# wondmgezahu/RAMP

Measured on AMD Instinct MI355X. Metric: sampled trajectories/sec (H=48, T=25), higher is better.
Workload: dtype f32-emulated (2 x fp16 planes per operand, fp32 accumulate)

## Files before the change

### ramp_amd/csrc/tkc.hip

```cpp
#include "args_conv.h"
#include "tokmma.h"

#include <algorithm>

namespace ramp {

namespace {

constexpr int tc_xrows(int NG) { return NG == 4 ? 64 + 2 + 2 : 48 + 2 * 6 + 2; }
constexpr int tc_scr(int NG) { return NG == 4 ? 2304 : 2048; }

__device__ __forceinline__ float tc_mish(float x) {
  const float e = __builtin_amdgcn_exp2f(fminf(x, 20.f) * 1.44269504088896340736f);
  const float n = e * (e + 2.f);
  return x * (n * __builtin_amdgcn_rcpf(n + 2.f));
}
__device__ __forceinline__ float tc_mish_grad(float x) {
  const float e = __builtin_amdgcn_exp2f(fminf(x, 20.f) * 1.44269504088896340736f);
  const float n = e * (e + 2.f);
  const float w = __builtin_amdgcn_rcpf(n + 2.f);
  return n * w + x * (4.f * e * (e + 1.f) * w * w);
}

__device__ __forceinline__ f32x4 tc_mm32(const u32x4 a, const u32x4 b, const f32x4 c) {
  return __builtin_amdgcn_mfma_f32_16x16x32_f16(__builtin_bit_cast(half8, a), __builtin_bit_cast(half8, b), c, 0, 0, 0);
}
__device__ __forceinline__ void tc_wave_sync() {
  __builtin_amdgcn_fence(__ATOMIC_ACQ_REL, "wavefront");
  __builtin_amdgcn_wave_barrier();
}

}

__global__ void tkc_pack_kernel(const float* __restrict__ W, unsigned short* __restrict__ out, int N, int K, float scale) {
  const int total = 5 * (N / 16) * (K / 32) * 64;
  const int idx = blockIdx.x * 256 + threadIdx.x;
  if (idx >= total) return;
  const int lane = idx & 63, f = idx >> 6;
  const int j = f % (K / 32), nb = (f / (K / 32)) % (N / 16), tap = f / ((K / 32) * (N / 16));
  const float* src = W + ((long)tap * N + 16 * nb + (lane & 15)) * K + 32 * j + 8 * (lane >> 4);
  unsigned short* o = out + (long)f * 1024 + lane * 8;
#pragma unroll
  for (int e = 0; e < 8; ++e) {
    const float x = src[e] * scale;
    const _Float16 hi = (_Float16)x, lo = (_Float16)(x - (float)hi);
    o[e] = __builtin_bit_cast(unsigned short, hi); o[512 + e] = __builtin_bit_cast(unsigned short, lo);
  }
}
int tkc_pack(const float* W, int N, int K, float scale, unsigned short* out, hipStream_t s) {
  RAMP_REQUIRE(W && out && N % 16 == 0 && K % 32 == 0 && N >= 16 && N <= 64 && K >= 32 && K <= 64, "tkc_pack: bad shape");
  const int total = 5 * (N / 16) * (K / 32) * 64;
  hipLaunchKernelGGL(tkc_pack_kernel, dim3((total + 255) / 256), dim3(256), 0, s, W, out, N, K, scale);
  RAMP_HIP_CHECK(hipGetLastError());
  return 0;
}
size_t tkc_packed_halves(int N, int K) { return (size_t)5 * (N / 16) * (K / 32) * 1024; }

template <int NG, int NB, int KS, int PRO, int EPI>
__global__ __launch_bounds__(256) __attribute__((amdgpu_waves_per_eu(1, 2)))
void tkc_kernel(TkcArgs a, int n_tiles) {
  constexpr int T = 16 * NG, K = 32 * KS, N = 16 * NB;
  constexpr int XROW = 4 * K + 16;
  constexpr int WBYTES = 5 * NB * KS * 2048;
  constexpr int TC_XROWS = tc_xrows(NG), TC_SCR = tc_scr(NG);
  static_assert(8 * T * 4 + 8 * (NG == 4 ? 1 : 6) * 4 <= TC_SCR, "GroupNorm scratch");
  extern __shared__ __attribute__((aligned(16))) char smem[];
  const int tid = threadIdx.x, lane = tid & 63;
  const int wave = __builtin_amdgcn_readfirstlane(tid >> 6);
  const int c = lane & 15, g = lane >> 4;
  const int n_my = (n_tiles - (int)blockIdx.x + (int)gridDim.x - 1) / (int)gridDim.x;

  const bool exact = a.amax_in == nullptr;
  float s_in = scale_of(a.amax_in);
  float os = a.wsi / s_in;
  float amax = 0.f;

  for (int i = tid; i < WBYTES / 16; i += 256) reinterpret_cast<u32x4*>(smem)[i] = reinterpret_cast<const u32x4*>(a.W)[i];
  char* xt = smem + WBYTES + wave * (TC_XROWS * XROW);
  for (int i = lane; i < TC_XROWS * XROW / 16; i += 64) reinterpret_cast<u32x4*>(xt)[i] = u32x4{0u, 0u, 0u, 0u};
  float* const wscr = reinterpret_cast<float*>(smem + WBYTES + 4 * (TC_XROWS * XROW) + wave * TC_SCR);
  __syncthreads();

  int xrow[NG], smp[NG];
#pragma unroll
  for (int t = 0; t < NG; ++t) { smp[t] = (16 * t + c) / a.L; xrow[t] = (16 * t + c) + 2 * smp[t] + 2; }
  const int n_smp = T / a.L;
  auto tok_sums = [&](float (&v)[4][NG], int nblk, int C) __attribute__((always_inline)) {
    const int gsz = C >> 3;
#pragma unroll
    for (int b = 0; b < 4; ++b) {
      if (b < nblk) {
#pragma unroll
        for (int t = 0; t < NG; ++t) {
          float q = v[b][t];
          if (gsz == 8) q += __shfl_xor(q, 16);
          const int grp = gsz == 4 ? 4 * b + g : 2 * b + (g >> 1);
          if (gsz == 4 || !(g & 1)) wscr[grp * T + 16 * t + c] = q;
        }
      }
    }
    tc_wave_sync();
    if (lane < 8 * n_smp) {
      const int grp = lane / n_smp, sm = lane - grp * n_smp;
      double q = 0.0;
      for (int u = 0; u < a.L; ++u) q += (double)wscr[grp * T + sm * a.L + u];
      wscr[8 * T + lane] = (float)(q / (double)(a.L * gsz));
    }
    tc_wave_sync();
#pragma unroll
    for (int b = 0; b < 4; ++b) {
      if (b < nblk) {
#pragma unroll
        for (int t = 0; t < NG; ++t) {
          const int grp = gsz == 4 ? 4 * b + g : 2 * b + (g >> 1);
          v[b][t] = wscr[8 * T + grp * n_smp + smp[t]];
        }
      }
    }
    tc_wave_sync();
  };
  const int m_last = a.M - 1;
  const char* xbase = reinterpret_cast<const char*>(a.X);

  f32x4 xr[K / 16][NG];
  f32x4 cr[PRO ? K / 16 : 1][PRO ? NG : 1];
  float gmu[PRO ? K / 16 : 1][PRO ? NG : 1], grs[PRO ? K / 16 : 1][PRO ? NG : 1];
  auto load_x = [&](int tile) __attribute__((always_inline)) {
    int tk0 = tile * (4 * T) + wave * T + c;
    asm volatile("" : "+v"(tk0));
#pragma unroll
    for (int t = 0; t < NG; ++t) {
      const unsigned tk = (unsigned)min(tk0 + 16 * t, m_last);
      const char* row = xbase + ((size_t)tk * (unsigned)(4 * a.ldx) + 16u * (unsigned)g);
#pragma unroll
      for (int fb = 0; fb < K / 16; ++fb) xr[fb][t] = *reinterpret_cast<const f32x4*>(row + 64 * fb);
      if constexpr (PRO) {
        const char* crow = reinterpret_cast<const char*>(a.gn_c) + ((size_t)tk * (unsigned)(4 * K) + 16u * (unsigned)g);
        const unsigned srow = tk / (unsigned)a.L;
// ... 13 lines not shown
      pgam[fb] = *reinterpret_cast<const f32x4*>(a.gn_gamma + 16 * fb + 4 * g); pbet[fb] = *reinterpret_cast<const f32x4*>(a.gn_beta + 16 * fb + 4 * g);
    }
  }
  load_x((int)blockIdx.x);

#pragma unroll 1
  for (int ti = 0; ti < n_my; ++ti) {
    const int tile = (int)blockIdx.x + ti * (int)gridDim.x;
    const int tile_n = ti + 1 < n_my ? tile + (int)gridDim.x : tile;
    const int tok0 = tile * (4 * T) + wave * T;
    const bool full = tok0 + T <= a.M;

    if constexpr (PRO) {
      float v1[4][NG], v2[4][NG];
#pragma unroll
      for (int fb = 0; fb < K / 16; ++fb)
#pragma unroll
        for (int t = 0; t < NG; ++t) {
          float s1 = 0.f, s2 = 0.f;
#pragma unroll
          for (int j = 0; j < 4; ++j) {
            const float h = (cr[fb][t][j] - gmu[fb][t]) * grs[fb][t];
            const float d = xr[fb][t][j] * tc_mish_grad(h * pgam[fb][j] + pbet[fb][j]) * pgam[fb][j];
            cr[fb][t][j] = h; xr[fb][t][j] = d;
            s1 += d; s2 += d * h;
          }
          v1[fb][t] = s1; v2[fb][t] = s2;
        }
      tok_sums(v1, K / 16, K);
      tok_sums(v2, K / 16, K);
#pragma unroll
      for (int fb = 0; fb < K / 16; ++fb)
#pragma unroll
        for (int t = 0; t < NG; ++t)
#pragma unroll
          for (int j = 0; j < 4; ++j) xr[fb][t][j] = (xr[fb][t][j] - v1[fb][t] - cr[fb][t][j] * v2[fb][t]) * grs[fb][t];
    }
    if (exact) {
      float tm = 0.f;
#pragma unroll
      for (int t = 0; t < NG; ++t) {
        const float lm = (full || tok0 + 16 * t + c < a.M) ? 1.f : 0.f;
#pragma unroll
        for (int fb = 0; fb < K / 16; ++fb) tm = amax4(xr[fb][t] * lm, tm);
      }
      tm = fmaxf(tm, __shfl_xor(tm, 32)); tm = fmaxf(tm, __shfl_xor(tm, 16)); tm = fmaxf(tm, __shfl_xor(tm, 8));
      tm = fmaxf(tm, __shfl_xor(tm, 4)); tm = fmaxf(tm, __shfl_xor(tm, 2)); tm = fmaxf(tm, __shfl_xor(tm, 1));
      s_in = scale_from(tm);
      os = a.wsi / s_in;
    }
#pragma unroll
    for (int t = 0; t < NG; ++t) {
      const float lm = (full || tok0 + 16 * t + c < a.M) ? 1.f : 0.f;
      char* dst = xt + xrow[t] * XROW + 8 * g;
#pragma unroll
      for (int fb = 0; fb < K / 16; ++fb) {
        const f32x4 v = xr[fb][t] * lm;
        amax = amax4(v, amax);
        unsigned h0, h1, l0, l1;
        split4(v * s_in, h0, h1, l0, l1);
        *reinterpret_cast<u32x2*>(dst + 32 * fb) = u32x2{h0, h1};
        *reinterpret_cast<u32x2*>(dst + 2 * K + 32 * fb) = u32x2{l0, l1};
      }
    }
    tc_wave_sync();
    load_x(tile_n);

    f32x4 acc[NB][NG];
#pragma unroll
    for (int nb = 0; nb < NB; ++nb)
#pragma unroll
      for (int t = 0; t < NG; ++t) acc[nb][t] = f32x4{0.f, 0.f, 0.f, 0.f};
#pragma unroll
    for (int tap = 0; tap < 5; ++tap) {
      const int sh = a.dir * (tap - 2);
#pragma unroll
      for (int j = 0; j < KS; ++j) {
        u32x4 bh[NG], bl[NG];
#pragma unroll
        for (int t = 0; t < NG; ++t) {
          const char* p = xt + (xrow[t] + sh) * XROW + 64 * j + 16 * g;
          bh[t] = *reinterpret_cast<const u32x4*>(p);
          bl[t] = *reinterpret_cast<const u32x4*>(p + 2 * K);
        }
#pragma unroll
        for (int nb = 0; nb < NB; ++nb) {
          const char* wp = smem + ((tap * NB + nb) * KS + j) * 2048 + lane * 16;
          const u32x4 wh = *reinterpret_cast<const u32x4*>(wp), wl = *reinterpret_cast<const u32x4*>(wp + 1024);
#pragma unroll
          for (int t = 0; t < NG; ++t) {
            f32x4 v = acc[nb][t];
            v = tc_mm32(wh, bl[t], v);
            v = tc_mm32(wl, bh[t], v);
            v = tc_mm32(wh, bh[t], v);
            acc[nb][t] = v;
          }
        }
      }
    }
    tc_wave_sync();

    if constexpr (EPI) {
      unsigned trow[NG];
#pragma unroll
      for (int t = 0; t < NG; ++t) trow[t] = (unsigned)min(tok0 + 16 * t + c, m_last);
      const float* tline[EPI == 2 ? NG : 1];
      if constexpr (EPI == 2) {
        const int s0 = tok0 / a.L, s_last = a.M / a.L - 1;
#pragma unroll
        for (int t = 0; t < NG; ++t) tline[t] = a.tbias + (size_t)a.t_rows[min(s0 + smp[t], s_last)] * (size_t)a.tt_stride + 4 * g;
      }
      float mean[4][NG], var[4][NG];
#pragma unroll
      for (int nb = 0; nb < NB; ++nb) {
        const f32x4 bq = *reinterpret_cast<const f32x4*>(a.bias + 16 * nb + 4 * g);
#pragma unroll
        for (int t = 0; t < NG; ++t) {
          acc[nb][t] = acc[nb][t] * os + bq;
          if (full || tok0 + 16 * t + c < a.M) *reinterpret_cast<f32x4*>(a.Cst + (size_t)trow[t] * N + 16 * nb + 4 * g) = acc[nb][t];
          mean[nb][t] = (acc[nb][t][0] + acc[nb][t][1]) + (acc[nb][t][2] + acc[nb][t][3]);
        }
      }
      tok_sums(mean, NB, N);
#pragma unroll
      for (int nb = 0; nb < NB; ++nb)
#pragma unroll
        for (int t = 0; t < NG; ++t) {
          float q = 0.f;
#pragma unroll
          for (int j = 0; j < 4; ++j) { const float d = acc[nb][t][j] - mean[nb][t]; q += d * d; }
          var[nb][t] = q;
        }
      tok_sums(var, NB, N);
#pragma unroll
// ... 26 lines not shown
#pragma unroll
      for (int nb = 0; nb < NB; ++nb) bq[nb] = a.bias ? *reinterpret_cast<const f32x4*>(a.bias + 16 * nb + 4 * g) : f32x4{0.f, 0.f, 0.f, 0.f};
      if (full) {
        f32x4 rz[NB][NG];
#pragma unroll
        for (int nb = 0; nb < NB; ++nb)
#pragma unroll
          for (int t = 0; t < NG; ++t) rz[nb][t] = f32x4{0.f, 0.f, 0.f, 0.f};
        if (a.resid) {
#pragma unroll
          for (int nb = 0; nb < NB; ++nb)
#pragma unroll
            for (int t = 0; t < NG; ++t) rz[nb][t] = *reinterpret_cast<const f32x4*>(a.resid + (size_t)trow[t] * a.ldr + 16 * nb + 4 * g);
        }
        if (a.resid2) {
#pragma unroll
          for (int nb = 0; nb < NB; ++nb)
#pragma unroll
            for (int t = 0; t < NG; ++t) rz[nb][t] += *reinterpret_cast<const f32x4*>(a.resid2 + (size_t)trow[t] * a.ldr2 + 16 * nb + 4 * g);
        }
#pragma unroll
        for (int nb = 0; nb < NB; ++nb)
#pragma unroll
          for (int t = 0; t < NG; ++t) *reinterpret_cast<f32x4*>(a.Y + (size_t)trow[t] * a.ldy + 16 * nb + 4 * g) = acc[nb][t] * os + bq[nb] + rz[nb][t];
      } else {
#pragma unroll
        for (int nb = 0; nb < NB; ++nb)
#pragma unroll
          for (int t = 0; t < NG; ++t) {
            f32x4 v = acc[nb][t] * os + bq[nb];
            if (a.resid) v += *reinterpret_cast<const f32x4*>(a.resid + (size_t)trow[t] * a.ldr + 16 * nb + 4 * g);
            if (a.resid2) v += *reinterpret_cast<const f32x4*>(a.resid2 + (size_t)trow[t] * a.ldr2 + 16 * nb + 4 * g);
            if (tok0 + 16 * t + c < a.M) *reinterpret_cast<f32x4*>(a.Y + (size_t)trow[t] * a.ldy + 16 * nb + 4 * g) = v;
          }
      }
    }
  }

    }
  amax = fmaxf(amax, __shfl_xor(amax, 32)); amax = fmaxf(amax, __shfl_xor(amax, 16)); amax = fmaxf(amax, __shfl_xor(amax, 8));
  amax = fmaxf(amax, __shfl_xor(amax, 4)); amax = fmaxf(amax, __shfl_xor(amax, 2)); amax = fmaxf(amax, __shfl_xor(amax, 1));
  __syncthreads();
  record_amax_block_guarded<true>(a.amax_out, amax, reinterpret_cast<float*>(smem + WBYTES), exact ? nullptr : a.range_flag, s_in, a.site);
}

bool tkc_applicable(int M, int L, int N, int K, int* ng) {
  int n = 0;
  if (L >= 8 && 48 % L == 0) n = 3; else if (L >= 8 && 32 % L == 0) n = 2; else if (L == 64 && !(N == 64 && K == 64)) n = 4;
  if (ng) *ng = n;
  return n != 0 && M > 0 && M % L == 0 && (N == 32 || N == 64) && (K == 32 || K == 64);
}

namespace {
template <int NG, int NB, int KS> size_t tkc_lds() { return (size_t)5 * NB * KS * 2048 + 4 * (size_t)tc_xrows(NG) * (4 * 32 * KS + 16) + 4 * tc_scr(NG); }
template <int NG, int NB, int KS, int PRO, int EPI> int tkc_go(const TkcArgs& a, int n_tiles, hipStream_t s) {
  const size_t lds = tkc_lds<NG, NB, KS>();
  const int per_cu = lds * 2 <= 160 * 1024 ? 2 : 1;
  const int nb = std::min(n_tiles, per_cu * device_cu_count());
  hipLaunchKernelGGL((tkc_kernel<NG, NB, KS, PRO, EPI>), dim3(nb), dim3(256), lds, s, a, n_tiles);
  RAMP_HIP_CHECK(hipGetLastError());
  return 0;
}
}

int launch_tkc(const TkcArgs& a, hipStream_t s) {
  auto al16 = [](const void* p) { return (reinterpret_cast<uintptr_t>(p) & 15) == 0; };
  int ng = 0;
  RAMP_REQUIRE(tkc_applicable(a.M, a.L, a.N, a.K, &ng), "tkc: C_in, C_out in {32, 64}, tokens per sample >= 8 dividing 48 or 32 (or 64, not 64 x 64 channels), whole samples");
  RAMP_REQUIRE(a.X && a.W && a.Y && (a.dir == 1 || a.dir == -1), "tkc: bad operand");
  RAMP_REQUIRE(al16(a.X) && al16(a.W) && al16(a.Y) && al16(a.bias) && al16(a.resid) && al16(a.resid2) && a.ldx % 4 == 0 && a.ldy % 4 == 0 &&
               a.ldr % 4 == 0 && a.ldr2 % 4 == 0 && a.ldx >= a.K && a.ldy >= a.N, "tkc: operands must be 16-byte aligned");
  RAMP_REQUIRE((long)a.M * a.ldx * 4 < (1l << 32), "tkc: 32-bit row offsets");
  RAMP_REQUIRE(!ranges_overlap(a.Y, ((size_t)(a.M - 1) * a.ldy + a.N) * 4, a.X, ((size_t)(a.M - 1) * a.ldx + a.K) * 4), "tkc: the output must not overlap the operand");
  const int T = 16 * ng, n_tiles = (a.M + 4 * T - 1) / (4 * T);
  const int pro = a.gn_c ? 1 : 0, epi = a.Cst ? (a.t_rows ? 2 : 1) : 0;
  RAMP_REQUIRE(!a.t_rows || (a.Cst && a.tbias && a.tt_stride > 0 && a.tt_stride % 4 == 0), "tkc: a row -> timestep table needs the GroupNorm epilogue, the time table and its stride (a multiple of 4 floats)");
  RAMP_REQUIRE(!(pro && epi), "tkc: the GroupNorm backward operand and the GroupNorm epilogue do not occur together");
  if (pro) RAMP_REQUIRE(a.gn_stats && a.gn_gamma && a.gn_beta && al16(a.gn_c) && al16(a.gn_gamma) && al16(a.gn_beta) && a.ldx >= a.K, "tkc: GroupNorm-backward operand incomplete");
  if (epi) RAMP_REQUIRE(a.stats && a.gamma && a.beta && a.bias && !a.resid2 && al16(a.Cst) && al16(a.gamma) && al16(a.beta) && al16(a.tbias), "tkc: GroupNorm epilogue incomplete");
#define TC_SHAPE(NGV, PROV, EPIV) \
    if (a.N == 64 && a.K == 64) return tkc_go<NGV, 4, 2, PROV, EPIV>(a, n_tiles, s); \
    if (a.N == 64 && a.K == 32) return tkc_go<NGV, 4, 1, PROV, EPIV>(a, n_tiles, s); \
    if (a.N == 32 && a.K == 64) return tkc_go<NGV, 2, 2, PROV, EPIV>(a, n_tiles, s); \
    return tkc_go<NGV, 2, 1, PROV, EPIV>(a, n_tiles, s);
#define TC_CASE(NGV) \
  if (ng == NGV) { \
    if (pro) { TC_SHAPE(NGV, 1, 0) } \
    if (epi == 2) { TC_SHAPE(NGV, 0, 2) } \
    if (epi) { TC_SHAPE(NGV, 0, 1) } \
    TC_SHAPE(NGV, 0, 0) \
  }
  TC_CASE(3) TC_CASE(2)
#undef TC_SHAPE
#define TC_SHAPE(NGV, PROV, EPIV) \
    if (a.N == 64 && a.K == 32) return tkc_go<NGV, 4, 1, PROV, EPIV>(a, n_tiles, s); \
    if (a.N == 32 && a.K == 64) return tkc_go<NGV, 2, 2, PROV, EPIV>(a, n_tiles, s); \
    if (a.N == 32 && a.K == 32) return tkc_go<NGV, 2, 1, PROV, EPIV>(a, n_tiles, s);
  TC_CASE(4)
#undef TC_CASE
#undef TC_SHAPE
  RAMP_REQUIRE(false, "tkc: variant not built");
}

int init_tkc_attributes() {
#define TC_ATTR1(NGV, NBV, KSV, PROV, EPIV) RAMP_HIP_CHECK(hipFuncSetAttribute(reinterpret_cast<const void*>(&tkc_kernel<NGV, NBV, KSV, PROV, EPIV>), hipFuncAttributeMaxDynamicSharedMemorySize, (int)tkc_lds<NGV, NBV, KSV>()))
#define TC_ATTR(NGV, NBV, KSV) TC_ATTR1(NGV, NBV, KSV, 0, 0); TC_ATTR1(NGV, NBV, KSV, 1, 0); TC_ATTR1(NGV, NBV, KSV, 0, 1); TC_ATTR1(NGV, NBV, KSV, 0, 2)
  TC_ATTR(3, 4, 2); TC_ATTR(3, 4, 1); TC_ATTR(3, 2, 2); TC_ATTR(3, 2, 1);
// ... 9 lines not shown
```

### ramp_amd/csrc/tkw.hip

```cpp
#include "args_conv.h"
#include "tokmma.h"

#include <algorithm>

namespace ramp {

namespace {

constexpr int TW_TB = 96;
constexpr int TW_NT = 3;
constexpr int TW_SCRATCH = 4096 + 4 * 1024;

__device__ __forceinline__ float tw_mish(float x) {
  const float e = __builtin_amdgcn_exp2f(fminf(x, 20.f) * 1.44269504088896340736f);
  const float n = e * (e + 2.f);
  return x * (n * __builtin_amdgcn_rcpf(n + 2.f));
}
__device__ __forceinline__ float tw_mish_grad(float x) {
  const float e = __builtin_amdgcn_exp2f(fminf(x, 20.f) * 1.44269504088896340736f);
  const float n = e * (e + 2.f);
  const float w = __builtin_amdgcn_rcpf(n + 2.f);
  return n * w + x * (4.f * e * (e + 1.f) * w * w);
}
__device__ __forceinline__ void tw_wave_sync() {
  __builtin_amdgcn_fence(__ATOMIC_ACQ_REL, "wavefront");
  __builtin_amdgcn_wave_barrier();
}

struct TwGeom { int KC, n_chunks, rows, xrow, n_pass; size_t lds; };
#define LR_GROUPS_OK(KC_, K_) (((KC_) / 4) / ((K_) / 32) <= 8)

}

template <int MB, int PRO, int EPI, bool RT>
__device__ __forceinline__ void tkw_body(const TkwArgs& a, int n_tiles, int kc32, int n_chunks, int n_rows, int n_pass, int mulL) {
  extern __shared__ __attribute__((aligned(16))) char smem[];
  const int tid = threadIdx.x, lane = tid & 63;
  const int wave = __builtin_amdgcn_readfirstlane(tid >> 6);
  const int tok = lane & 31, kh = lane >> 5;
  const int KC = kc32 << 5;
  const int XROW = 4 * KC + 16;
  const int KS = KC >> 4;
  char* const scr = smem + (size_t)n_rows * XROW;
  float* const wscr = reinterpret_cast<float*>(scr + wave * 1024);

  const float s_in = scale_of(a.amax_in);
  const float os = a.wsi / s_in;
  float amax = 0.f;
  auto divL = [&](int t) __attribute__((always_inline)) { return (t * mulL) >> 16; };
  auto trow = [&](int t) __attribute__((always_inline)) { return t + 2 * divL(t) + 2; };

  for (int i = tid; i < n_rows * XROW / 16; i += 256) reinterpret_cast<u32x4*>(smem)[i] = u32x4{0u, 0u, 0u, 0u};
  float* const prm = reinterpret_cast<float*>(scr + 4096);
  auto load_prm = [&](int c0) __attribute__((always_inline)) {
    for (int i = tid; i < min(a.N, 256); i += 256) {
      const int c = c0 + i;
      prm[i] = a.bias[c]; prm[256 + i] = a.gamma[c]; prm[512 + i] = a.beta[c]; prm[768 + i] = a.tbias ? a.tbias[c] : 0.f;
    }
  };
  if (EPI >= 1) load_prm(0);
  __syncthreads();

  int boff[TW_NT];
#pragma unroll
  for (int tg = 0; tg < TW_NT; ++tg) boff[tg] = trow(32 * tg + tok) * XROW + 16 * kh;
  const int LR = KC >> 2;
  const int RP = 64 / LR;
  const int sl = lane % LR, sr = lane / LR;
  const int m_last = a.M - 1;

#pragma unroll 1
  for (int tile = (int)blockIdx.x; tile < n_tiles; tile += (int)gridDim.x) {
    const int tok0 = tile * TW_TB;
#pragma unroll 1
    for (int pass = 0; pass < n_pass; ++pass) {
      f32x16 acc[MB][TW_NT];
#pragma unroll
      for (int mb = 0; mb < MB; ++mb)
#pragma unroll
        for (int tg = 0; tg < TW_NT; ++tg)
#pragma unroll
          for (int i = 0; i < 16; ++i) acc[mb][tg][i] = 0.f;
      const int nb0 = pass * 128 * MB + wave * 32 * MB;

#pragma unroll 1
      for (int kc = 0; kc < n_chunks; ++kc) {
        if (pass > 0 || kc > 0 || tile != (int)blockIdx.x) __syncthreads();
        if (EPI == 2 && kc == 0 && (pass > 0 || tile != (int)blockIdx.x)) load_prm(pass * 256);
        if (n_chunks > 1 || pass == 0) {
          const int ch = kc * KC + 4 * sl;
          if constexpr (PRO == 0) {
#pragma unroll 1
            for (int it0 = 0; it0 < 24; it0 += 8 * RP) {
              f32x4 v[8];
#pragma unroll
              for (int u = 0; u < 8; ++u) {
                const int t = 24 * wave + it0 + u * RP + sr;
                const int tk = min(tok0 + t, m_last);
                const float* src = ch < a.K1 ? a.X + (size_t)tk * a.ldx + ch : a.X2 + (size_t)tk * a.ldx2 + (ch - a.K1);
                v[u] = (it0 + u * RP < 24 && !(a.ablate & 2)) ? *reinterpret_cast<const f32x4*>(src) : f32x4{0.f, 0.f, 0.f, 0.f};
              }
#pragma unroll
              for (int u = 0; u < 8; ++u) {
                if (it0 + u * RP < 24) {
                  const int t = 24 * wave + it0 + u * RP + sr;
                  const f32x4 x = (tok0 + t < a.M) ? v[u] : f32x4{0.f, 0.f, 0.f, 0.f};
                  amax = amax4(x, amax);
                  unsigned h0, h1, l0, l1;
                  split4(x * s_in, h0, h1, l0, l1);
                  char* dst = smem + trow(t) * XROW + 8 * sl;
                  *reinterpret_cast<u32x2*>(dst) = u32x2{h0, h1};
                  *reinterpret_cast<u32x2*>(dst + 2 * KC) = u32x2{l0, l1};
                }
              }
            }
          } else {
            constexpr int NW = PRO > 0 ? PRO : 1;
            const int G4 = (a.K >> 5);
            const int grp = ch / (a.K >> 3), gl = sl / G4;
            const int n_gl = LR / G4;
            const f32x4 gam = *reinterpret_cast<const f32x4*>(a.gn_gamma + ch), bet = *reinterpret_cast<const f32x4*>(a.gn_beta + ch);
            const float inv_cnt = 1.f / (float)(a.L * (a.K >> 3));
            const int n_it = a.L / RP;
            const int spp = NW / n_it;
            const int n_smp = TW_TB / a.L;
            const int sm_lo = (wave * n_smp) >> 2, sm_hi = ((wave + 1) * n_smp) >> 2;
#pragma unroll 1
            for (int sm0 = sm_lo; sm0 < sm_hi; sm0 += spp) {
              const int t_lo = sm0 * a.L;
              f32x4 dv[NW], hv[NW];
              float mu[NW], rs[NW];
              int u_s = 0, u_i = 0;
#pragma unroll
              for (int u = 0; u < NW; ++u) {
                const int tk = min(tok0 + t_lo + u * RP + sr, m_last);
                dv[u] = *reinterpret_cast<const f32x4*>(a.X + (size_t)tk * a.ldx + ch);
                hv[u] = *reinterpret_cast<const f32x4*>(a.gn_c + (size_t)tk * a.K + ch);
                const int srow = min(tok0 / a.L + sm0 + u_s, m_last / a.L);
                mu[u] = a.gn_stats[((size_t)srow * 8 + grp) * 2]; rs[u] = a.gn_stats[((size_t)srow * 8 + grp) * 2 + 1];
                if (++u_i == n_it) { u_i = 0; ++u_s; }
              }
              float p1[NW], p2[NW];
#pragma unroll
              for (int u = 0; u < NW; ++u) {
                float s1 = 0.f, s2 = 0.f;
#pragma unroll
                for (int j = 0; j < 4; ++j) {
                  const float h = (hv[u][j] - mu[u]) * rs[u];
                  const float d = dv[u][j] * tw_mish_grad(h * gam[j] + bet[j]) * gam[j];
                  hv[u][j] = h; dv[u][j] = d;
                  s1 += d; s2 += d * h;
                }
                p1[u] = s1; p2[u] = s2;
              }
              for (int b = 1; b < G4; b <<= 1) {
#pragma unroll
                for (int u = 0; u < NW; ++u) { p1[u] += __shfl_xor(p1[u], b); p2[u] += __shfl_xor(p2[u], b); }
              }
              for (int b = LR; b < 64; b <<= 1) {
#pragma unroll
                for (int u = 0; u < NW; ++u) { p1[u] += __shfl_xor(p1[u], b); p2[u] += __shfl_xor(p2[u], b); }
              }
              if (sr == 0 && sl == gl * G4) {
#pragma unroll
                for (int u = 0; u < NW; ++u) { wscr[(gl * 8 + u) * 2] = p1[u]; wscr[(gl * 8 + u) * 2 + 1] = p2[u]; }
              }
              tw_wave_sync();
              if (lane < n_gl * spp) {
                const int g2 = lane / spp, s2i = lane - g2 * spp;
                float t1 = 0.f, t2 = 0.f;
                for (int i2 = 0; i2 < n_it; ++i2) { t1 += wscr[(g2 * 8 + s2i * n_it + i2) * 2]; t2 += wscr[(g2 * 8 + s2i * n_it + i2) * 2 + 1]; }
                wscr[(g2 * 8 + s2i * n_it) * 2] = t1 * inv_cnt; wscr[(g2 * 8 + s2i * n_it) * 2 + 1] = t2 * inv_cnt;
              }
              tw_wave_sync();
              u_s = 0; u_i = 0;
#pragma unroll
              for (int u = 0; u < NW; ++u) {
                const float m1 = wscr[(gl * 8 + u_s * n_it) * 2], m2 = wscr[(gl * 8 + u_s * n_it) * 2 + 1];
                if (++u_i == n_it) { u_i = 0; ++u_s; }
                const int t = t_lo + u * RP + sr;
                const bool live = tok0 + t < a.M;
                f32x4 x;
#pragma unroll
                for (int j = 0; j < 4; ++j) x[j] = live ? (dv[u][j] - m1 - hv[u][j] * m2) * rs[u] : 0.f;
                amax = amax4(x, amax);
                unsigned h0, h1, l0, l1;
                split4(x * s_in, h0, h1, l0, l1);
                char* dst = smem + trow(t) * XROW + 8 * sl;
                *reinterpret_cast<u32x2*>(dst) = u32x2{h0, h1};
                *reinterpret_cast<u32x2*>(dst + 2 * KC) = u32x2{l0, l1};
              }
              tw_wave_sync();
            }
          }
        }
        __syncthreads();

        const int n_steps = 5 * KS;
        const int lks = 31 - __builtin_clz(KS);
        const size_t wtap = (size_t)(a.N >> 5) * (a.K >> 4) * 2048;
        const char* wbase = reinterpret_cast<const char*>(a.W) + ((size_t)(nb0 >> 5) * (a.K >> 4) + (size_t)kc * KS) * 2048 + lane * 16;
        const size_t wmb = (size_t)(a.K >> 4) * 2048;
        auto load_a = [&](u32x4 (&h)[MB], u32x4 (&l)[MB], int st) __attribute__((always_inline)) {
          const char* p = wbase + (size_t)(st >> lks) * wtap + (size_t)(st & (KS - 1)) * 2048;
#pragma unroll
          for (int mb = 0; mb < MB; ++mb) {
            h[mb] = *reinterpret_cast<const u32x4*>(p + mb * wmb);
            l[mb] = *reinterpret_cast<const u32x4*>(p + mb * wmb + 1024);
          }
        };
        auto load_b = [&](u32x4 (&h)[TW_NT], u32x4 (&l)[TW_NT], int st) __attribute__((always_inline)) {
          const int sh = a.dir * ((st >> lks) - 2) * XROW + 32 * (st & (KS - 1));
#pragma unroll
          for (int tg = 0; tg < TW_NT; ++tg) {
            const char* p = smem + boff[tg] + sh;
            h[tg] = *reinterpret_cast<const u32x4*>(p);
            l[tg] = *reinterpret_cast<const u32x4*>(p + 2 * KC);
          }
        };
        auto step = [&](const u32x4 (&uah)[MB], const u32x4 (&ual)[MB], const u32x4 (&ubh)[TW_NT], const u32x4 (&ubl)[TW_NT],
                        u32x4 (&nah)[MB], u32x4 (&nal)[MB], u32x4 (&nbh)[TW_NT], u32x4 (&nbl)[TW_NT], int nxt) __attribute__((always_inline)) {
          const int sc = min(nxt, n_steps - 1);
          const char* pa = wbase + (size_t)(sc >> lks) * wtap + (size_t)(sc & (KS - 1)) * 2048;
          const int shn = a.dir * ((sc >> lks) - 2) * XROW + 32 * (sc & (KS - 1));
          auto issue = [&](int q) __attribute__((always_inline)) {
            if (q < 2 * MB) {
              const u32x4 v = *reinterpret_cast<const u32x4*>(pa + (q >> 1) * wmb + (q & 1) * 1024);
              if (q & 1) nal[q >> 1] = v; else nah[q >> 1] = v;
            } else if (q < 2 * MB + 2 * TW_NT) {
              const int r = q - 2 * MB;
              const u32x4 v = *reinterpret_cast<const u32x4*>(smem + boff[r >> 1] + shn + (r & 1) * 2 * KC);
              if (r & 1) nbl[r >> 1] = v; else nbh[r >> 1] = v;
            }
          };
          int q = 0;
#pragma unroll
          for (int mb = 0; mb < MB; ++mb)
#pragma unroll
            for (int tg = 0; tg < TW_NT; ++tg) {
              f32x16 v = acc[mb][tg];
              v = mfma16(uah[mb], ubl[tg], v);
              issue(q++);
              __builtin_amdgcn_sched_barrier(0);
              v = mfma16(ual[mb], ubh[tg], v);
              issue(q++);
              __builtin_amdgcn_sched_barrier(0);
              v = mfma16(uah[mb], ubh[tg], v);
              issue(q++);
              __builtin_amdgcn_sched_barrier(0);
              acc[mb][tg] = v;
            }
        };
        u32x4 a0h[MB], a0l[MB], a1h[MB], a1l[MB], b0h[TW_NT], b0l[TW_NT], b1h[TW_NT], b1l[TW_NT];
        load_a(a0h, a0l, 0); load_b(b0h, b0l, 0);
        __builtin_amdgcn_sched_barrier(0);
#pragma unroll 1
        for (int st = (a.ablate & 1) ? n_steps : 0; st < n_steps; st += 2) {
          step(a0h, a0l, b0h, b0l, a1h, a1l, b1h, b1l, st + 1);
          step(a1h, a1l, b1h, b1l, a0h, a0l, b0h, b0l, st + 2);
        }
      }

      if (EPI == 0) {
#pragma unroll
        for (int tg = 0; tg < TW_NT; ++tg) {
          const int t = tok0 + 32 * tg + tok;
          const int tk = min(t, m_last);
#pragma unroll
          for (int mb = 0; mb < MB; ++mb)
#pragma unroll
            for (int q = 0; q < 4; ++q) {
              const int n = nb0 + 32 * mb + 8 * q + 4 * kh;
              f32x4 v = quad(acc[mb][tg], q) * os;
              if (a.bias) v += *reinterpret_cast<const f32x4*>(a.bias + n);
              if (a.resid) v += *reinterpret_cast<const f32x4*>(a.resid + (size_t)tk * a.ldr + n);
              if (a.resid2) v += *reinterpret_cast<const f32x4*>(a.resid2 + (size_t)tk * a.ldr2 + n);
              float* dst = n < a.N1 ? a.Y + (size_t)tk * a.ldy + n : a.Y2 + (size_t)tk * a.ldy2 + (n - a.N1);
              if (t < a.M && !(a.ablate & 4)) *reinterpret_cast<f32x4*>(dst) = v;
            }
        }
      } else {
        constexpr int NGW = EPI == 2 ? 1 : 2;
        const int poff = EPI == 2 ? pass * 256 : 0;
        const int gsz = a.N >> 3;
// ... 73 lines not shown
          if (tok0 + sm * a.L < a.M) {
            const int g = EPI == 2 ? (nb0 >> 6) : (nb0 >> 5) * (MB == 2 ? 1 : 2) + gi;
            float* st = a.stats + ((size_t)(tok0 / a.L + sm) * 8 + g) * 2;
            st[0] = my_mean; st[1] = 1.f / sqrtf(my_var + a.eps);
          }
        }
#pragma unroll
        for (int tg = 0; tg < TW_NT; ++tg) {
          const int t = tok0 + 32 * tg + tok;
          const int tk = min(t, m_last);
          const float* tline = nullptr;
          if constexpr (RT) tline = a.tbias + (size_t)a.t_rows[min(tok0 / a.L + divL(32 * tg + tok), m_last / a.L)] * (size_t)a.tt_stride;
#pragma unroll
          for (int mb = 0; mb < MB; ++mb)
#pragma unroll
            for (int q = 0; q < 4; ++q) {
              const int n = nb0 + 32 * mb + 8 * q + 4 * kh;
              const int gi = EPI == 2 ? 0 : MB == 2 ? mb : (q >> 1);
              const f32x4 gam = *reinterpret_cast<const f32x4*>(prm + 256 + n - poff), bet = *reinterpret_cast<const f32x4*>(prm + 512 + n - poff);
              f32x4 v;
#pragma unroll
              for (int j = 0; j < 4; ++j) v[j] = tw_mish((acc[mb][tg][4 * q + j] - mean_t[gi][tg]) * rstd_t[gi][tg] * gam[j] + bet[j]);
              if constexpr (RT) v += *reinterpret_cast<const f32x4*>(tline + n);
              else v += *reinterpret_cast<const f32x4*>(prm + 768 + n - poff);
              if (a.resid) v += *reinterpret_cast<const f32x4*>(a.resid + (size_t)tk * a.ldr + n);
              if (t < a.M && !(a.ablate & 4)) *reinterpret_cast<f32x4*>(a.Y + (size_t)tk * a.ldy + n) = v;
            }
        }
      }
    }
  }

  amax = fmaxf(amax, __shfl_xor(amax, 32)); amax = fmaxf(amax, __shfl_xor(amax, 16)); amax = fmaxf(amax, __shfl_xor(amax, 8));
  amax = fmaxf(amax, __shfl_xor(amax, 4)); amax = fmaxf(amax, __shfl_xor(amax, 2)); amax = fmaxf(amax, __shfl_xor(amax, 1));
  record_amax_block_guarded<true>(a.amax_out, amax, reinterpret_cast<float*>(scr), a.range_flag, s_in, a.site);
}

template <int PRO, int EPI>
__global__ __launch_bounds__(256) __attribute__((amdgpu_waves_per_eu(2, 2)))
void tkw_kernel1(TkwArgs a, int n_tiles, int kc32, int n_chunks, int n_rows, int n_pass, int mulL) { tkw_body<1, PRO, EPI, false>(a, n_tiles, kc32, n_chunks, n_rows, n_pass, mulL); }
template <int PRO, int EPI>
__global__ __launch_bounds__(256) __attribute__((amdgpu_waves_per_eu(2, 2)))
void tkw_kernel2(TkwArgs a, int n_tiles, int kc32, int n_chunks, int n_rows, int n_pass, int mulL) { tkw_body<2, PRO, EPI, false>(a, n_tiles, kc32, n_chunks, n_rows, n_pass, mulL); }
template <int MB, int EPI>
__global__ __launch_bounds__(256) __attribute__((amdgpu_waves_per_eu(2, 2)))
void tkw_rows_kernel(TkwArgs a, int n_tiles, int kc32, int n_chunks, int n_rows, int n_pass, int mulL) { tkw_body<MB, 0, EPI, true>(a, n_tiles, kc32, n_chunks, n_rows, n_pass, mulL); }

namespace {

bool tw_geometry(int L, int N, int K, TwGeom* g) {
  if (L < 3 || TW_TB % L != 0) return false;
  if (!(N == 128 || N == 256 || N == 512 || N == 1024)) return false;
  if (K < 32 || K > 1024 || (K & (K - 1)) != 0) return false;
  const int rows = TW_TB + 2 * (TW_TB / L + 1);
  int KC = std::min(K, 128);
  while (KC > 32 && (size_t)rows * (4 * KC + 16) + TW_SCRATCH > 80 * 1024) KC >>= 1;
  if (KC < 32 || K % KC != 0) return false;
  g->KC = KC; g->n_chunks = K / KC; g->rows = rows; g->xrow = 4 * KC + 16;
  g->n_pass = N <= 256 ? 1 : N / 256;
  g->lds = (size_t)rows * g->xrow + TW_SCRATCH;
  return g->lds <= 80 * 1024;
}

int tw_pro_variant(int L, int N, int K) {
  TwGeom g;
  if (!tw_geometry(L, N, K, &g)) return 0;
  const int RP = 64 / (g.KC / 4);
  if (L % RP != 0 || (K / 8) % 4 != 0) return 0;
  const int n_it = L / RP, n_smp = TW_TB / L;
  for (int nw : {6, 8, 4, 3}) {
    if (nw % n_it != 0) continue;
    const int spp = nw / n_it;
    bool ok = true;
    for (int w = 0; w < 4; ++w) ok &= ((((w + 1) * n_smp) >> 2) - ((w * n_smp) >> 2)) % spp == 0;
    if (ok && (LR_GROUPS_OK(g.KC, K))) return nw;
  }
  return 0;
}

template <int MB, int PRO, int EPI, bool RT = false> int tkw_go(const TkwArgs& a, const TwGeom& g, hipStream_t s) {
  const int n_tiles = (a.M + TW_TB - 1) / TW_TB;
  const int per_cu = g.lds * 2 <= 160 * 1024 ? 2 : 1;
  const int nb = std::min(n_tiles, per_cu * device_cu_count());
  if constexpr (RT) hipLaunchKernelGGL((tkw_rows_kernel<MB, EPI ? EPI : 1>), dim3(nb), dim3(256), g.lds, s, a, n_tiles, g.KC >> 5, g.n_chunks, g.rows, g.n_pass, (65536 + a.L - 1) / a.L);
  else if (MB == 1) hipLaunchKernelGGL((tkw_kernel1<PRO, EPI>), dim3(nb), dim3(256), g.lds, s, a, n_tiles, g.KC >> 5, g.n_chunks, g.rows, g.n_pass, (65536 + a.L - 1) / a.L);
  else hipLaunchKernelGGL((tkw_kernel2<PRO, EPI>), dim3(nb), dim3(256), g.lds, s, a, n_tiles, g.KC >> 5, g.n_chunks, g.rows, g.n_pass, (65536 + a.L - 1) / a.L);
  RAMP_HIP_CHECK(hipGetLastError());
  return 0;
}

}

namespace { int tw_pro_variant(int L, int N, int K); }
bool tkw_applicable(int M, int L, int N, int K, int pro, int epi) {
  TwGeom g;
  if (!(M > 0 && M % L == 0 && tw_geometry(L, N, K, &g))) return false;
  if ((long)M * std::max(N, K) * 4 >= (1l << 32)) return false;
  if (pro) {
    if (tw_pro_variant(L, N, K) == 0) return false;
    if (g.n_chunks > 1 && (K / 8) > g.KC) return false;
  }
  if (epi && N > 512) return false;
  return true;
}

int launch_tkw(const TkwArgs& a, hipStream_t s) {
  auto al16 = [](const void* p) { return (reinterpret_cast<uintptr_t>(p) & 15) == 0; };
  const int pro = a.gn_c ? 1 : 0, epi = a.Cst ? 1 : 0;
  TwGeom g;
  RAMP_REQUIRE(tkw_applicable(a.M, a.L, a.N, a.K, pro, epi) && tw_geometry(a.L, a.N, a.K, &g),
               "tkw: C_out in {128, 256, 512, 1024} (<= 512 with the GroupNorm epilogue), C_in a power of two in [32, 1024], tokens per sample >= 3 dividing 96 (24 with the GroupNorm backward), whole samples");
  RAMP_REQUIRE(a.X && a.W && a.Y && (a.dir == 1 || a.dir == -1), "tkw: bad operand");
  RAMP_REQUIRE(a.K1 == a.K || (a.X2 && a.K1 > 0 && a.K1 < a.K && a.K1 % 4 == 0 && !pro), "tkw: bad operand split");
// ... 37 lines not shown
```

Baseline: 4228.

## Replace per-sample halo rows with shared zero block and per-lane tap masks

```diff
diff --git a/ramp_amd/csrc/conv_tile.h b/ramp_amd/csrc/conv_tile.h
--- /dev/null
+++ b/ramp_amd/csrc/conv_tile.h
@@ -0,0 +1,75 @@
+#pragma once
+
+#if defined(__HIPCC__) || defined(__CUDACC__)
+#define CT_HD __host__ __device__ __forceinline__
+#else
+#define CT_HD inline
+#endif
+
+namespace ramp {
+
+constexpr int CT_TAPS = 5;
+constexpr int CT_WIDE_TOKENS = 96, CT_WIDE_GROUPS = 3;
+
+CT_HD constexpr int ct_pitch_wide(int kc) { return 4 * kc + 16; }
+CT_HD constexpr int ct_pitch_narrow(int k) { return 4 * k + 32; }
+CT_HD constexpr int ct_zero_rows(int pitch) {
+  int z = 16;
+  for (int q = (pitch >> 4) & 15; z > 1 && !(q & 1); q >>= 1) z >>= 1;
+  return z;
+}
+constexpr int CT_Z_WIDE = 16, CT_Z_NARROW = 8;
+static_assert(ct_zero_rows(ct_pitch_wide(32)) == CT_Z_WIDE && ct_zero_rows(ct_pitch_wide(64)) == CT_Z_WIDE && ct_zero_rows(ct_pitch_wide(128)) == CT_Z_WIDE,
+              "tkw: the pitch is an odd number of 16-byte quads");
+static_assert(ct_zero_rows(ct_pitch_narrow(32)) == CT_Z_NARROW && ct_zero_rows(ct_pitch_narrow(64)) == CT_Z_NARROW, "tkc: the pitch is twice an odd number of quads");
+
+CT_HD constexpr int ct_tile_rows(int z, int tokens) { return z + tokens; }
+CT_HD constexpr int ct_tile_bytes(int pitch, int z, int tokens) { return ct_tile_rows(z, tokens) * pitch; }
+
+constexpr int CT_WIDE_SCRATCH = 4096 + 4 * 1024;
+CT_HD constexpr int ct_wide_lds(int kc) { return ct_tile_bytes(ct_pitch_wide(kc), CT_Z_WIDE, CT_WIDE_TOKENS) + CT_WIDE_SCRATCH; }
+CT_HD constexpr int ct_narrow_scratch(int ng) { return ng == 4 ? 2304 : 2048; }
+CT_HD constexpr int ct_narrow_lds(int ng, int nb, int ks) {
+  return 5 * nb * ks * 2048 + 4 * ct_tile_bytes(ct_pitch_narrow(32 * ks), CT_Z_NARROW, 16 * ng) + 4 * ct_narrow_scratch(ng);
+}
+
+CT_HD constexpr int ct_stage_addr(int pitch, int kc, int z, int t, int ch, int plane) { return (z + t) * pitch + 2 * ch + plane * 2 * kc; }
+
+CT_HD constexpr unsigned ct_tap_mask(int pos, int L, int dir) {
+  unsigned m = 0;
+  for (int j = 0; j < CT_TAPS; ++j) m |= ((unsigned)(pos + dir * (j - 2)) < (unsigned)L ? 1u : 0u) << j;
+  return m;
+}
+CT_HD constexpr int ct_tap_row(int z, int t, unsigned m, int j, int dir) {
+  const int u = t + dir * (j - 2);
+  return ((m >> j) & 1u) ? z + u : (u & (z - 1));
+}
+CT_HD constexpr int ct_frag_addr(int pitch, int kc, int row, int c0, int plane) { return row * pitch + 2 * c0 + plane * 2 * kc; }
+
+CT_HD constexpr unsigned ct_wide_masks(int lane, int L, int dir) {
+  unsigned m = 0;
+  for (int tg = 0; tg < CT_WIDE_GROUPS; ++tg) m |= ct_tap_mask((32 * tg + (lane & 31)) % L, L, dir) << (CT_TAPS * tg);
+  return m;
+}
+CT_HD constexpr unsigned ct_wide_lane(int kc, int lane, int L, int dir) {
+  return (unsigned)(lane >> 5) << 31 | ct_wide_masks(lane, L, dir) << 16 | (unsigned)ct_frag_addr(ct_pitch_wide(kc), kc, CT_Z_WIDE + (lane & 31), 8 * (lane >> 5), 0);
+}
+CT_HD constexpr int ct_wide_read(int kc, unsigned pk, int tok, int tg, int tap, int ks, int dir, int plane) {
+  const int pitch = ct_pitch_wide(kc), d = dir * (tap - 2);
+  const int col = 32 * ks + plane * 2 * kc;
+  const int data = (int)(pk & 0xffffu) + ((32 * tg + d) * pitch + col);
+  const int zero = ((tok + d) & (CT_Z_WIDE - 1)) * pitch + ((int)(pk >> 31) * 16 + col);
+  return (pk & (1u << (16 + CT_TAPS * tg + tap))) ? data : zero;
+}
+
+CT_HD constexpr unsigned ct_narrow_masks(int lane, int ng, int L, int dir) {
+  unsigned m = 0;
+  for (int t = 0; t < ng; ++t) m |= ct_tap_mask((16 * t + (lane & 15)) % L, L, dir) << (CT_TAPS * t);
+  return m;
+}
+CT_HD constexpr int ct_narrow_read(int k, int lane, unsigned masks, int t, int tap, int j, int dir, int plane) {
+  const int row = ct_tap_row(CT_Z_NARROW, 16 * t + (lane & 15), masks >> (CT_TAPS * t), tap, dir);
+  return ct_frag_addr(ct_pitch_narrow(k), k, row, 32 * j + 8 * (lane >> 4), plane);
+}
+
+}
diff --git a/ramp_amd/csrc/tkc.hip b/ramp_amd/csrc/tkc.hip
--- a/ramp_amd/csrc/tkc.hip
+++ b/ramp_amd/csrc/tkc.hip
@@ -1,4 +1,5 @@
 #include "args_conv.h"
+#include "conv_tile.h"
 #include "tokmma.h"
 
 #include <algorithm>
@@ -7,8 +8,8 @@
 
 namespace {
 
-constexpr int tc_xrows(int NG) { return NG == 4 ? 64 + 2 + 2 : 48 + 2 * 6 + 2; }
-constexpr int tc_scr(int NG) { return NG == 4 ? 2304 : 2048; }
+constexpr int tc_xrows(int NG) { return ct_tile_rows(CT_Z_NARROW, 16 * NG); }
+constexpr int tc_scr(int NG) { return ct_narrow_scratch(NG); }
 
 __device__ __forceinline__ float tc_mish(float x) {
   const float e = __builtin_amdgcn_exp2f(fminf(x, 20.f) * 1.44269504088896340736f);
@@ -60,7 +61,7 @@
 __global__ __launch_bounds__(256) __attribute__((amdgpu_waves_per_eu(1, 2)))
 void tkc_kernel(TkcArgs a, int n_tiles) {
   constexpr int T = 16 * NG, K = 32 * KS, N = 16 * NB;
-  constexpr int XROW = 4 * K + 16;
+  constexpr int XROW = ct_pitch_narrow(K);
   constexpr int WBYTES = 5 * NB * KS * 2048;
   constexpr int TC_XROWS = tc_xrows(NG), TC_SCR = tc_scr(NG);
   static_assert(8 * T * 4 + 8 * (NG == 4 ? 1 : 6) * 4 <= TC_SCR, "GroupNorm scratch");
@@ -77,13 +78,14 @@
 
   for (int i = tid; i < WBYTES / 16; i += 256) reinterpret_cast<u32x4*>(smem)[i] = reinterpret_cast<const u32x4*>(a.W)[i];
   char* xt = smem + WBYTES + wave * (TC_XROWS * XROW);
-  for (int i = lane; i < TC_XROWS * XROW / 16; i += 64) reinterpret_cast<u32x4*>(xt)[i] = u32x4{0u, 0u, 0u, 0u};
+  for (int i = lane; i < CT_Z_NARROW * XROW / 16; i += 64) reinterpret_cast<u32x4*>(xt)[i] = u32x4{0u, 0u, 0u, 0u};
   float* const wscr = reinterpret_cast<float*>(smem + WBYTES + 4 * (TC_XROWS * XROW) + wave * TC_SCR);
   __syncthreads();
 
-  int xrow[NG], smp[NG];
-#pragma unroll
-  for (int t = 0; t < NG; ++t) { smp[t] = (16 * t + c) / a.L; xrow[t] = (16 * t + c) + 2 * smp[t] + 2; }
+  int smp[NG];
+#pragma unroll
+  for (int t = 0; t < NG; ++t) smp[t] = (16 * t + c) / a.L;
+  const unsigned tmask = ct_narrow_masks(lane, NG, a.L, a.dir);
   const int n_smp = T / a.L;
   auto tok_sums = [&](float (&v)[4][NG], int nblk, int C) __attribute__((always_inline)) {
     const int gsz = C >> 3;
@@ -203,7 +205,7 @@
 #pragma unroll
     for (int t = 0; t < NG; ++t) {
       const float lm = (full || tok0 + 16 * t + c < a.M) ? 1.f : 0.f;
-      char* dst = xt + xrow[t] * XROW + 8 * g;
+      char* dst = xt + ct_stage_addr(XROW, K, CT_Z_NARROW, 16 * t + c, 4 * g, 0);
 #pragma unroll
       for (int fb = 0; fb < K / 16; ++fb) {
         const f32x4 v = xr[fb][t] * lm;
@@ -224,13 +226,12 @@
       for (int t = 0; t < NG; ++t) acc[nb][t] = f32x4{0.f, 0.f, 0.f, 0.f};
 #pragma unroll
     for (int tap = 0; tap < 5; ++tap) {
-      const int sh = a.dir * (tap - 2);
 #pragma unroll
       for (int j = 0; j < KS; ++j) {
         u32x4 bh[NG], bl[NG];
 #pragma unroll
         for (int t = 0; t < NG; ++t) {
-          const char* p = xt + (xrow[t] + sh) * XROW + 64 * j + 16 * g;
+          const char* p = xt + ct_narrow_read(K, lane, tmask, t, tap, j, a.dir, 0);
           bh[t] = *reinterpret_cast<const u32x4*>(p);
           bl[t] = *reinterpret_cast<const u32x4*>(p + 2 * K);
         }
@@ -363,7 +364,7 @@
 }
 
 namespace {
-template <int NG, int NB, int KS> size_t tkc_lds() { return (size_t)5 * NB * KS * 2048 + 4 * (size_t)tc_xrows(NG) * (4 * 32 * KS + 16) + 4 * tc_scr(NG); }
+template <int NG, int NB, int KS> size_t tkc_lds() { return (size_t)ct_narrow_lds(NG, NB, KS); }
 template <int NG, int NB, int KS, int PRO, int EPI> int tkc_go(const TkcArgs& a, int n_tiles, hipStream_t s) {
   const size_t lds = tkc_lds<NG, NB, KS>();
   const int per_cu = lds * 2 <= 160 * 1024 ? 2 : 1;
diff --git a/ramp_amd/csrc/tkw.hip b/ramp_amd/csrc/tkw.hip
--- a/ramp_amd/csrc/tkw.hip
+++ b/ramp_amd/csrc/tkw.hip
@@ -1,4 +1,5 @@
 #include "args_conv.h"
+#include "conv_tile.h"
 #include "tokmma.h"
 
 #include <algorithm>
@@ -9,7 +10,7 @@
 
 constexpr int TW_TB = 96;
 constexpr int TW_NT = 3;
-constexpr int TW_SCRATCH = 4096 + 4 * 1024;
+constexpr int TW_SCRATCH = CT_WIDE_SCRATCH;
 
 __device__ __forceinline__ float tw_mish(float x) {
   const float e = __builtin_amdgcn_exp2f(fminf(x, 20.f) * 1.44269504088896340736f);
@@ -39,7 +40,7 @@
   const int wave = __builtin_amdgcn_readfirstlane(tid >> 6);
   const int tok = lane & 31, kh = lane >> 5;
   const int KC = kc32 << 5;
-  const int XROW = 4 * KC + 16;
+  const int XROW = ct_pitch_wide(KC);
   const int KS = KC >> 4;
   char* const scr = smem + (size_t)n_rows * XROW;
   float* const wscr = reinterpret_cast<float*>(scr + wave * 1024);
@@ -48,9 +49,8 @@
   const float os = a.wsi / s_in;
   float amax = 0.f;
   auto divL = [&](int t) __attribute__((always_inline)) { return (t * mulL) >> 16; };
-  auto trow = [&](int t) __attribute__((always_inline)) { return t + 2 * divL(t) + 2; };
-
-  for (int i = tid; i < n_rows * XROW / 16; i += 256) reinterpret_cast<u32x4*>(smem)[i] = u32x4{0u, 0u, 0u, 0u};
+
+  for (int i = tid; i < CT_Z_WIDE * XROW / 16; i += 256) reinterpret_cast<u32x4*>(smem)[i] = u32x4{0u, 0u, 0u, 0u};
   float* const prm = reinterpret_cast<float*>(scr + 4096);
   auto load_prm = [&](int c0) __attribute__((always_inline)) {
     for (int i = tid; i < min(a.N, 256); i += 256) {
@@ -61,9 +61,7 @@
   if (EPI >= 1) load_prm(0);
   __syncthreads();
 
-  int boff[TW_NT];
-#pragma unroll
-  for (int tg = 0; tg < TW_NT; ++tg) boff[tg] = trow(32 * tg + tok) * XROW + 16 * kh;
+  const unsigned bpk = ct_wide_lane(KC, lane, a.L, a.dir);
   const int LR = KC >> 2;
   const int RP = 64 / LR;
   const int sl = lane % LR, sr = lane / LR;
@@ -108,9 +106,8 @@
                   amax = amax4(x, amax);
                   unsigned h0, h1, l0, l1;
                   split4(x * s_in, h0, h1, l0, l1);
-                  char* dst = smem + trow(t) * XROW + 8 * sl;
-                  *reinterpret_cast<u32x2*>(dst) = u32x2{h0, h1};
-                  *reinterpret_cast<u32x2*>(dst + 2 * KC) = u32x2{l0, l1};
+                  *reinterpret_cast<u32x2*>(smem + ct_stage_addr(XROW, KC, CT_Z_WIDE, t, 4 * sl, 0)) = u32x2{h0, h1};
+                  *reinterpret_cast<u32x2*>(smem + ct_stage_addr(XROW, KC, CT_Z_WIDE, t, 4 * sl, 1)) = u32x2{l0, l1};
                 }
               }
             }
@@ -186,9 +183,8 @@
                 amax = amax4(x, amax);
                 unsigned h0, h1, l0, l1;
                 split4(x * s_in, h0, h1, l0, l1);
-                char* dst = smem + trow(t) * XROW + 8 * sl;
-                *reinterpret_cast<u32x2*>(dst) = u32x2{h0, h1};
-                *reinterpret_cast<u32x2*>(dst + 2 * KC) = u32x2{l0, l1};
+                *reinterpret_cast<u32x2*>(smem + ct_stage_addr(XROW, KC, CT_Z_WIDE, t, 4 * sl, 0)) = u32x2{h0, h1};
+                *reinterpret_cast<u32x2*>(smem + ct_stage_addr(XROW, KC, CT_Z_WIDE, t, 4 * sl, 1)) = u32x2{l0, l1};
               }
               tw_wave_sync();
             }
@@ -210,10 +206,9 @@
           }
         };
         auto load_b = [&](u32x4 (&h)[TW_NT], u32x4 (&l)[TW_NT], int st) __attribute__((always_inline)) {
-          const int sh = a.dir * ((st >> lks) - 2) * XROW + 32 * (st & (KS - 1));
 #pragma unroll
           for (int tg = 0; tg < TW_NT; ++tg) {
-            const char* p = smem + boff[tg] + sh;
+            const char* p = smem + ct_wide_read(KC, bpk, tok, tg, st >> lks, st & (KS - 1), a.dir, 0);
             h[tg] = *reinterpret_cast<const u32x4*>(p);
             l[tg] = *reinterpret_cast<const u32x4*>(p + 2 * KC);
           }
@@ -222,14 +217,14 @@
                         u32x4 (&nah)[MB], u32x4 (&nal)[MB], u32x4 (&nbh)[TW_NT], u32x4 (&nbl)[TW_NT], int nxt) __attribute__((always_inline)) {
           const int sc = min(nxt, n_steps - 1);
           const char* pa = wbase + (size_t)(sc >> lks) * wtap + (size_t)(sc & (KS - 1)) * 2048;
-          const int shn = a.dir * ((sc >> lks) - 2) * XROW + 32 * (sc & (KS - 1));
+          const int ntap = sc >> lks, nks = sc & (KS - 1);
           auto issue = [&](int q) __attribute__((always_inline)) {
             if (q < 2 * MB) {
               const u32x4 v = *reinterpret_cast<const u32x4*>(pa + (q >> 1) * wmb + (q & 1) * 1024);
               if (q & 1) nal[q >> 1] = v; else nah[q >> 1] = v;
             } else if (q < 2 * MB + 2 * TW_NT) {
               const int r = q - 2 * MB;
-              const u32x4 v = *reinterpret_cast<const u32x4*>(smem + boff[r >> 1] + shn + (r & 1) * 2 * KC);
+              const u32x4 v = *reinterpret_cast<const u32x4*>(smem + ct_wide_read(KC, bpk, tok, r >> 1, ntap, nks, a.dir, 0) + (r & 1) * 2 * KC);
               if (r & 1) nbl[r >> 1] = v; else nbh[r >> 1] = v;
             }
           };
@@ -409,13 +404,12 @@
   if (L < 3 || TW_TB % L != 0) return false;
   if (!(N == 128 || N == 256 || N == 512 || N == 1024)) return false;
   if (K < 32 || K > 1024 || (K & (K - 1)) != 0) return false;
-  const int rows = TW_TB + 2 * (TW_TB / L + 1);
+  const int rows = ct_tile_rows(CT_Z_WIDE, TW_TB);
   int KC = std::min(K, 128);
-  while (KC > 32 && (size_t)rows * (4 * KC + 16) + TW_SCRATCH > 80 * 1024) KC >>= 1;
   if (KC < 32 || K % KC != 0) return false;
-  g->KC = KC; g->n_chunks = K / KC; g->rows = rows; g->xrow = 4 * KC + 16;
+  g->KC = KC; g->n_chunks = K / KC; g->rows = rows; g->xrow = ct_pitch_wide(KC);
   g->n_pass = N <= 256 ? 1 : N / 256;
-  g->lds = (size_t)rows * g->xrow + TW_SCRATCH;
+  g->lds = (size_t)ct_wide_lds(KC);
   return g->lds <= 80 * 1024;
 }
 
```

Result: slower. 4154 (-1.8%).
